# OnurBasci/TransformerBasedNavierStokeSolver

Measured on AMD Instinct MI355X. Metric: ns64_train_samples_per_s, higher is better.
Workload: dtype f32

## Files before the change

transformerbasednavierstokesolver_amd/csrc/pa2d_gemm.hip:

```cpp
#include "pa2d_gemm_common.h"
#include <string.h>


static Pa2dEnv read_env() {
    auto is = [](const char* n, const char* pre) { const char* e = getenv(n); return e && strncmp(e, pre, strlen(pre)) == 0; };
    auto num = [](const char* n, int dflt) { const char* e = getenv(n); return (e && e[0]) ? atoi(e) : dflt; };
    Pa2dEnv v;
    v.conv_halo = is("PA2D_CONV_HALO", "o") ? 0 : (is("PA2D_CONV_HALO", "f") ? 2 : 1);
    v.mc_big_off = is("PA2D_MC_BIG", "o") ? 1 : 0;
    v.kc_bk16 = num("PA2D_KC_BK", 0) == 16 ? 1 : 0;
    v.mc_bk = num("PA2D_MC_BK", 16) == 32 ? 32 : 16;
    v.mc_splits = num("PA2D_MC_SPLITS", 0);
    v.mcb_splits = num("PA2D_MCB_SPLITS", 0);
    v.lin_dw_split = is("PA2D_LIN_DW_SPLIT", "of") ? 0 : 1;
    v.lin_panel = is("PA2D_LIN_PANEL", "of") ? 0 : 1;
    v.lin_rowpanel = is("PA2D_LIN_ROWPANEL", "of") ? 0 : 1;
    v.lin_small_split = is("PA2D_LIN_SMALL_SPLIT", "of") ? 0 : 1;
    v.conv_mfma16 = num("PA2D_CONV_MFMA", 16) == 32 ? 0 : 1;
    v.conv_ahead = num("PA2D_CONV_AHEAD", 1) == 0 ? 0 : 1;
    v.mc_mfma16 = num("PA2D_MC_MFMA", 16) == 32 ? 0 : 1;
    v.mc_dma = num("PA2D_MC_DMA", 1) == 0 ? 0 : 1;
    v.mc_chain = num("PA2D_MC_CHAIN", 1) == 0 ? 0 : 1;
    v.split_big = num("PA2D_SPLIT_BIG", 1);
    v.slice_map = is("PA2D_SLICE_MAP", "l") ? 0 : 1;
    v.default_engine = is("PA2D_GEMM", "f") ? 0 : (is("PA2D_GEMM", "b") ? 2 : 1);
    v.tail_panel = num("PA2D_TAIL_PANEL", 0);
    return v;
}
static Pa2dEnv g_env = read_env();
const Pa2dEnv& pa2d_env() { return g_env; }


static int kc_bk(bool im2col, int Cin) {
    if (im2col && pa2d_env().kc_bk16) return 16;
    return (!im2col || (Cin % 32) == 0) ? 32 : 16;
}
static KCTile kc_tile(int M, int N, bool im2col, int Cin) {
    const int tiles_m = ceil_div(M, 128);
    const long long t128 = (long long)tiles_m * ceil_div(N, 128);
    const long long t12864 = (long long)tiles_m * ceil_div(N, 64);
    const int bk = kc_bk(im2col, Cin);
    if (N > 64 && t128 >= 384) return {128, 128, bk};
    if (t12864 >= 384 || M <= 64) return {128, 64, bk};
    return {64, 64, bk};
}
static bool use_split(int engine, int N, bool im2col, int Cin) {
    const int m = engine;
    if (m == 1) return im2col && N > 64 && (Cin % 32) == 0;
    if (m == 2) return N > 64 && (!im2col || (Cin % 32) == 0);
    return false;
}
static bool kc_split_small_applies(const KCParams& p, bool im2col) {
    if (!pa2d_env().lin_small_split || im2col || p.io_bf16 || p.engine != 1) return false;
    if ((p.K % 32) != 0 || p.K < 64 || p.N < 64 || p.M < 256) return false;
    return (long long)ceil_div(p.M, 128) * ceil_div(p.N, 128) < 384;
}
static int persistent_mode(const KCParams& p) {
    const bool gelu = p.act == ACT_GELU, has_res = p.res != nullptr;
    if (p.epi == 0) return 0;
    if (gelu && !has_res && (p.epi == (EPI_ACT | EPI_STORE_PRE) || p.epi == EPI_ACT)) return 1;
    if (gelu && !has_res && p.epi == EPI_MUL_DACT && !p.bias) return 2;
    return -1;
}
static bool panel_applies(const KCParams& p, bool im2col) {
    if (!pa2d_env().lin_panel || im2col) return false;
    if (p.io_bf16 || (p.engine != 1 && p.engine != 2)) return false;
    if ((p.K % 32) != 0 || p.N < 64) return false;
    if (persistent_mode(p) < 0) return false;
    if (p.epi == EPI_ACT && p.aux) return false;
    return (long long)(p.M / 256) * ceil_div(p.N, 128) >= 256;
}
static size_t rowpanel_image_bytes(int N, int K, int engine) {
    if (engine != 1 || (K != 128 && K != 256) || N < 128 || N > 1024 || (N % 128) != 0) return 0;
    return (size_t)N * K * 6;
}
static bool rowpanel_applies(const KCParams& p) {
    if (!pa2d_env().lin_rowpanel || p.io_bf16) return false;
    if (rowpanel_image_bytes(p.N, p.K, p.engine) == 0) return false;
    if (persistent_mode(p) < 0 || (p.epi == EPI_ACT && p.aux)) return false;
    if ((p.lda & 3) || (p.ldc & 3) || (p.res && (p.ldres & 3)) || (p.aux && (p.ldaux & 3))) return false;
    return p.M / 128 >= 256;
}
static bool conv_halo_applies(const KCParams& p) {
    const int pol = pa2d_env().conv_halo;
    if (p.taps == 27) return false;
    if (pol == 0 || !p.apre || (p.Cin % 32) != 0 || p.H <= 0 || p.W <= 0 || (p.M % (p.H * p.W)) != 0) return false;
    const long long tiles = (long long)(p.M / (p.H * p.W)) * ceil_div(p.H, KC_HALO_TH) * ceil_div(p.W, KC_HALO_TW) * ceil_div(p.N, 128);
    return pol == 2 || tiles >= 512;
}

KCChoice plan_kc(const KCParams& p, bool im2col) {
    KCChoice c = {};
    c.mode = c.tail_family = c.tail_bm = c.tail_bn = -1;
    c.out_bf16 = p.io_bf16;
    c.reads_b = true;
    c.wimg_bytes = im2col ? 0 : rowpanel_image_bytes(p.N, p.K, p.engine);
    const int nt = p.engine == 2 ? 1 : 3;
    if (!im2col && p.wimg && rowpanel_applies(p)) {
        c.family = KC_ROWPANEL; c.bm = 128; c.bn = 64; c.bk = 64; c.nt = 3;
    } else if (panel_applies(p, im2col)) {
        c.family = KC_PANEL; c.bm = 256; c.bn = 128; c.bk = 32; c.nt = nt;
    } else if (p.io_bf16 || use_split(p.engine, p.N, im2col, p.Cin)) {
        c.family = KC_SPLIT; c.bm = 128; c.bn = 128; c.bk = 32; c.nt = nt;
        c.a_planes = im2col ? p.apre != 0 : p.io_bf16 != 0;
        if (im2col) c.pack = KC_PACK_PLANES;
        if (im2col ? !p.apre : p.engine != 2) c.rc = PA2D_ERR_ARG;
        else if (p.io_bf16 && (p.taps == 27 || p.engine != 2 || (!im2col && (p.K % 32) != 0))) c.rc = PA2D_ERR_UNSUPPORTED;
        else if (im2col && conv_halo_applies(p)) {
            c.family = KC_HALO; c.bm = 256;
            c.mfma16 = nt == 3 && pa2d_env().conv_mfma16 && (p.N % 4) == 0 && (p.ldc % 4) == 0;
            c.ahead = c.mfma16 && pa2d_env().conv_ahead;
        } else if (im2col && !p.io_bf16 && nt == 3) {
            const int tiles_n = ceil_div(p.N, 128);
            if (pa2d_env().split_big && (p.M % 256) == 0 && (long long)(p.M / 256) * tiles_n >= 512) c.bm = 256;
            else if ((long long)ceil_div(p.M, 128) * tiles_n < 256) c.bm = 64;
        }
    } else if (kc_split_small_applies(p, im2col)) {
        c.family = KC_SPLIT_SMALL; c.bm = 64; c.bn = 64; c.bk = 32; c.nt = 3;
    } else {
        const KCTile t = kc_tile(p.M, p.N, im2col, p.Cin);
        c.family = KC_EXACT; c.bm = t.bm; c.bn = t.bn; c.bk = t.bk;
        if (im2col) c.pack = t.bk == 32 ? KC_PACK_F32_32 : KC_PACK_F32_16;
    }
    if (c.family == KC_PANEL || c.family == KC_ROWPANEL) {
        c.mode = persistent_mode(p);
        c.head_rows = p.M - p.M % c.bm;
        if (c.head_rows < p.M) {
            KCParams pt = p;
            pt.wimg = nullptr;
            pt.M = p.M - c.head_rows;
            const KCChoice t = plan_kc(pt, false);
            c.tail_family = t.family; c.tail_bm = t.bm; c.tail_bn = t.bn;
        }
        c.reads_b = c.family == KC_PANEL || c.head_rows < p.M;
    }
    return c;
}

static bool kc_extents(KCParams& p, bool im2col, const KCChoice& c) {
    const unsigned long long lim = 0xFFFFFFF0ull;
    const unsigned long long es = p.io_bf16 ? 2ull : 4ull;
    unsigned long long ab = ((unsigned long long)(p.M - 1) * p.lda + (im2col ? p.Cin : p.K)) * 4ull;
    unsigned long long bb = ((unsigned long long)(p.N - 1) * p.ldb + p.K) * 4ull;
    const unsigned long long cb = ((unsigned long long)(p.M - 1) * p.ldc + p.N) * es;
    const unsigned long long rb = p.res ? ((unsigned long long)(p.M - 1) * p.ldres + p.N) * es : 0ull;
    const unsigned long long xb = p.aux ? ((unsigned long long)(p.M - 1) * p.ldaux + p.N) * es : 0ull;
    if (ab >= lim || bb >= lim || cb >= lim || rb >= lim || xb >= lim) return false;
    if (c.a_planes) ab = im2col ? (unsigned long long)p.M * (p.Cin / 32) * c.nt * 64 : ab / 2;
    if (c.pack == KC_PACK_PLANES) bb = (unsigned long long)p.N * (p.K / 32) * c.nt * 64;
    if (ab >= lim) return false;
    p.a_bytes = (unsigned)ab; p.b_bytes = (unsigned)bb;
    p.c_bytes = (unsigned)cb; p.res_bytes = (unsigned)rb; p.aux_bytes = (unsigned)xb;
    return true;
}

static int launch_head_tail(const KCParams& p_in, const KCParams& p, const KCChoice& c, hipStream_t st) {
    int rc;
    if (c.family == KC_ROWPANEL && p.wsrc) {
        rc = launch_pack_weight_image(p.wsrc, p.wsn, p.wsk, p.wimg, p.N, p.K, st);
        if (rc) return rc;
    }
    KCParams ph = p;
    ph.M = c.head_rows;
    rc = c.family == KC_ROWPANEL ? launch_kc_rowpanel(ph, c, st) : launch_kc_panel(ph, c, st);
    if (rc || c.head_rows == p.M) return rc;
    KCParams pt = p_in;
    pt.wimg = nullptr;
    pt.M = p.M - c.head_rows;
    pt.A = p.A + (size_t)c.head_rows * p.lda;
    pt.C = p.C + (size_t)c.head_rows * p.ldc;
    if (p.res) pt.res = p.res + (size_t)c.head_rows * p.ldres;
    if (p.aux) pt.aux = p.aux + (size_t)c.head_rows * p.ldaux;
    return launch_kc(pt, false, st);
}

// ... 258 lines not shown
```

transformerbasednavierstokesolver_amd/csrc/pa2d_gemm_rowpanel.hip:

```cpp
#include "pa2d_gemm_common.h"
#include <type_traits>
#ifndef RP_SGB
#define RP_SGB 1
#endif

namespace {

constexpr int RP_STAGE = 24 * 1024;
constexpr int RP_SLOTS = 3;
constexpr int RP_BIAS = 4096;

typedef unsigned int u32x4_ __attribute__((ext_vector_type(4)));

__device__ __forceinline__ float4 ld4s(__amdgpu_buffer_rsrc_t r, unsigned voff, unsigned soff) {
    const u32x4_ v = __builtin_amdgcn_raw_buffer_load_b128(r, voff, soff, 0);
    return make_float4(__uint_as_float(v.x), __uint_as_float(v.y), __uint_as_float(v.z), __uint_as_float(v.w));
}
__device__ __forceinline__ void st4s(__amdgpu_buffer_rsrc_t r, unsigned voff, unsigned soff, const float (&v)[4]) {
    const u32x4_ u = {__float_as_uint(v[0]), __float_as_uint(v[1]), __float_as_uint(v[2]), __float_as_uint(v[3])};
    __builtin_amdgcn_raw_buffer_store_b128(u, r, voff, soff, 0);
}
__device__ __forceinline__ bf16x8 cat8(bf16x4 a, bf16x4 b) { return __builtin_shufflevector(a, b, 0, 1, 2, 3, 4, 5, 6, 7); }

__global__ void pack_weight_image_kernel(const float* __restrict__ src, long long sn, long long sk, unsigned char* __restrict__ img,
                                         int N, int K) {
    const int idx = blockIdx.x * blockDim.x + threadIdx.x;
    const int KC = K / 64;
    if (idx >= (N / 64) * KC * 8 * 64) return;
    const int lane = idx & 63, j = (idx >> 6) & 1, sub = (idx >> 7) & 3, stage = idx >> 9;
    const int np = stage / KC, kc = stage % KC;
    const int n = 64 * np + 16 * (2 * (sub & 1) + j) + (lane & 15), k0 = 64 * kc + 32 * (sub >> 1) + 8 * (lane >> 4);
    float v[8];
#pragma unroll
    for (int e = 0; e < 8; ++e) v[e] = src[(long long)n * sn + (long long)(k0 + e) * sk];
    bf16x4 h0, m0, l0, h1, m1, l1;
    split3(make_float4(v[0], v[1], v[2], v[3]), h0, m0, l0);
    split3(make_float4(v[4], v[5], v[6], v[7]), h1, m1, l1);
    unsigned char* dst = img + (size_t)stage * RP_STAGE + (size_t)((sub * 2 + j) * 3) * 1024 + lane * 16;
    *reinterpret_cast<bf16x8*>(dst) = cat8(h0, h1);
    *reinterpret_cast<bf16x8*>(dst + 1024) = cat8(m0, m1);
    *reinterpret_cast<bf16x8*>(dst + 2048) = cat8(l0, l1);
}

template <int KS, int MODE, bool HAS_RES>
__global__ __launch_bounds__(256, 1) void gemm_rowpanel_kernel(const KCParams p, const unsigned char* __restrict__ img,
                                                               const unsigned img_bytes) {
    constexpr int KC = KS / 4;
    extern __shared__ __attribute__((aligned(16))) unsigned char smem[];
    const int tid = threadIdx.x, lane = tid & 63;
    const int wave = __builtin_amdgcn_readfirstlane(tid >> 6);
    const int li = lane & 15, kq = lane >> 4;
    const int NP = p.N / 64, SPR = NP * KC;
    float* const bias_s = reinterpret_cast<float*>(smem);
    unsigned char* const ring = smem + RP_BIAS;
    for (int c = tid; c < p.N; c += 256)
        bias_s[c] = (MODE != 2 && p.bias) ? (c < p.bias_split ? p.bias[c] : p.bias2[c - p.bias_split]) : 0.f;
    const int rounds = p.M / 128;
    const int n_my = ((int)blockIdx.x < rounds) ? (rounds - (int)blockIdx.x + (int)gridDim.x - 1) / (int)gridDim.x : 0;
    if (n_my == 0) return;
    const int T = n_my * SPR;

    const __amdgpu_buffer_rsrc_t ra = make_rsrc(p.A, p.a_bytes);
    const __amdgpu_buffer_rsrc_t ri = make_rsrc_v(img, img_bytes);
    const __amdgpu_buffer_rsrc_t rc = make_rsrc(p.C, p.c_bytes);
    const __amdgpu_buffer_rsrc_t rres = make_rsrc(p.res ? p.res : p.C, p.res ? p.res_bytes : 0u);
    const __amdgpu_buffer_rsrc_t raux = make_rsrc(p.aux ? p.aux : p.C, p.aux ? p.aux_bytes : 0u);
    const unsigned lda_b = (unsigned)p.lda * 4u, ldc_b = (unsigned)p.ldc * 4u, ldres_b = (unsigned)p.ldres * 4u,
                   ldaux_b = (unsigned)p.ldaux * 4u;

    const unsigned piece = (unsigned)(wave * 6) * 1024u + (unsigned)lane * 16u;
    u32x4_ breg[6];
    int ld_stage = 0;
    auto stage_load = [&]() {
#pragma unroll
        for (int i = 0; i < 6; ++i)
            breg[i] = __builtin_amdgcn_raw_buffer_load_b128(ri, piece + i * 1024u, (unsigned)ld_stage * RP_STAGE, 0);
        if (++ld_stage == SPR) ld_stage = 0;
    };
    auto stage_write = [&](int slot) {
#pragma unroll
        for (int i = 0; i < 6; ++i) *reinterpret_cast<u32x4_*>(ring + slot * RP_STAGE + piece + i * 1024) = breg[i];
    };

    const unsigned a_voff = (unsigned)li * lda_b + (unsigned)kq * 32u;
    float4 raw[KS][2];
    bf16x8 ap[KS][3];
    auto a_load = [&](int u, unsigned voff, unsigned row0) {
        const unsigned so = (row0 + 16u * (u & 1)) * lda_b;
        raw[u][0] = ld4s(ra, voff == OOB_OFF ? OOB_OFF : voff + (u >> 1) * 128u, so);
        raw[u][1] = ld4s(ra, voff == OOB_OFF ? OOB_OFF : voff + (u >> 1) * 128u + 16u, so);
    };
    auto a_split = [&](int ks) {
        bf16x4 h0, m0, l0, h1, m1, l1;
        split3(raw[ks][0], h0, m0, l0);
        split3(raw[ks][1], h1, m1, l1);
        ap[ks][0] = cat8(h0, h1); ap[ks][1] = cat8(m0, m1); ap[ks][2] = cat8(l0, l1);
    };

    int round = blockIdx.x;
    unsigned row0 = (unsigned)(round * 128 + wave * 32);
#pragma unroll
    for (int ks = 0; ks < KS; ++ks) a_load(ks, a_voff, row0);
    stage_load();
    stage_write(0);
    stage_load();
#pragma unroll
    for (int ks = 0; ks < KS; ++ks) a_split(ks);
    __syncthreads();

    const unsigned vc = li * ldc_b + kq * 16u, vr = li * ldres_b + kq * 16u, vx = li * ldaux_b + kq * 16u;

    bf16x8 bfb[2][2][3];
    int cur = 0;
    auto frag_read = [&](int buf, int slot, int ks4) {
        const unsigned char* bs = ring + slot * RP_STAGE + lane * 16;
#pragma unroll
        for (int j = 0; j < 2; ++j)
#pragma unroll
            for (int u = 0; u < 3; ++u) bfb[buf][j][u] = *reinterpret_cast<const bf16x8*>(bs + ((ks4 * 2 + j) * 3 + u) * 1024);
    };
    frag_read(0, 0, 0);

    f32x4 acc[2][4];
    float4 ov[2][4];
    auto ep_group = [&](const int q8, const int np) {
        const int rb = q8 >> 2, nt = q8 & 3;
        const unsigned cb = (unsigned)(np * 64 + nt * 16) * 4u;
        const unsigned rw = row0 + 16u * rb;
        float v[4];
#pragma unroll
        for (int e = 0; e < 4; ++e) v[e] = acc[rb][nt][e];
        if (MODE == 1) {
            if (p.aux_deriv) {
                float d[4];
#pragma unroll
                for (int e = 0; e < 4; ++e) d[e] = dgelu_f(v[e]);
                st4s(raux, vx, rw * ldaux_b + cb, d);
            } else {
                st4s(raux, vx, rw * ldaux_b + cb, v);
            }
#pragma unroll
            for (int e = 0; e < 4; ++e) v[e] = gelu_f(v[e]);
        } else if (MODE == 2) {
            if (p.aux_deriv) {
                v[0] *= ov[rb][nt].x; v[1] *= ov[rb][nt].y; v[2] *= ov[rb][nt].z; v[3] *= ov[rb][nt].w;
            } else {
                v[0] *= dgelu_f(ov[rb][nt].x); v[1] *= dgelu_f(ov[rb][nt].y); v[2] *= dgelu_f(ov[rb][nt].z); v[3] *= dgelu_f(ov[rb][nt].w);
            }
        } else if (HAS_RES) {
            v[0] += ov[rb][nt].x; v[1] += ov[rb][nt].y; v[2] += ov[rb][nt].z; v[3] += ov[rb][nt].w;
        }
#ifdef RP_NO_STORE
        if (p.M == 12345)
#endif
        st4s(rc, vc, rw * ldc_b + cb, v);
    };
    auto ov_load = [&](const int q8, const int np) {
        const int rb = q8 >> 2, nt = q8 & 3;
        const unsigned cb = (unsigned)(np * 64 + nt * 16) * 4u;
        if (MODE == 2) ov[rb][nt] = ld4s(raux, vx, (row0 + 16u * rb) * ldaux_b + cb);
        else if (HAS_RES) ov[rb][nt] = ld4s(rres, vr, (row0 + 16u * rb) * ldres_b + cb);
    };

    unsigned row0n = 0, a_voff_n = OOB_OFF;
    auto pair = [&](auto first_tag, auto last_tag, const int np) {
        constexpr bool FIRST = decltype(first_tag)::value, LAST = decltype(last_tag)::value;
#pragma unroll
        for (int nt = 0; nt < 4; ++nt) {
            const float4 bv = *reinterpret_cast<const float4*>(bias_s + np * 64 + nt * 16 + 4 * kq);
#pragma unroll
            for (int rb = 0; rb < 2; ++rb) {
                acc[rb][nt] = f32x4{bv.x, bv.y, bv.z, bv.w};
                ov_load(rb * 4 + nt, np);
            }
        }
#pragma unroll
        for (int kc = 0; kc < KC; ++kc) {
            const int nxt = cur == 2 ? 0 : cur + 1;
#ifndef RP_NO_BSTAGE
            stage_write(nxt);
            stage_load();
#endif
#ifndef RP_NO_ANEXT
            if (FIRST) {
#pragma unroll
                for (int q = 0; q < 4; ++q) a_load(kc * 4 + q, a_voff_n, row0n);
            }
#endif
#pragma unroll
            for (int ks4 = 0; ks4 < 4; ++ks4) {
                if (ks4 < 3) frag_read((ks4 + 1) & 1, cur, ks4 + 1);
                else frag_read(0, nxt, 0);
#if RP_SGB == 2
                __builtin_amdgcn_sched_barrier(0);
#endif
                const int ks = kc * 4 + ks4;
#ifndef RP_NO_ANEXT
                if (LAST && kc >= 1) a_split(ks - 4);
                if (FIRST && kc == 0) a_split(KS - 4 + ks4);
#endif
#define RP_MFMA(u_, v_)                                                                                      \
    _Pragma("unroll") for (int j = 0; j < 2; ++j) _Pragma("unroll") for (int rb = 0; rb < 2; ++rb)            \
        acc[rb][2 * (ks4 & 1) + j] = __builtin_amdgcn_mfma_f32_16x16x32_bf16(                                 \
            bfb[ks4 & 1][j][v_], ap[kc * 4 + (ks4 >> 1) * 2 + rb][u_], acc[rb][2 * (ks4 & 1) + j], 0, 0, 0);
#ifndef RP_NO_MFMA
                RP_MFMA(1, 1) RP_MFMA(2, 0) RP_MFMA(0, 2) RP_MFMA(1, 0) RP_MFMA(0, 1) RP_MFMA(0, 0)
#endif
#undef RP_MFMA
#if RP_SGB == 1
#pragma unroll
                for (int i = 0; i < 6; ++i) {
                    __builtin_amdgcn_sched_group_barrier(0x008, 4, 0);
                    __builtin_amdgcn_sched_group_barrier(0x100, 1, 0);
                }
#endif
#ifndef RP_NO_BARRIER
                if (ks4 == 1) __syncthreads();
#endif
            }
            cur = nxt;
        }
#pragma unroll
        for (int q8 = 0; q8 < 8; ++q8) ep_group(q8, np);
    };
    using T_ = std::true_type; using F_ = std::false_type;

    for (int t = 0; t < n_my; ++t) {
        const bool more = t + 1 < n_my;
        row0n = more ? (unsigned)((round + (int)gridDim.x) * 128 + wave * 32) : 0u;
        a_voff_n = more ? a_voff : OOB_OFF;
        pair(T_{}, F_{}, 0);
        for (int np = 1; np < NP - 1; ++np) pair(F_{}, F_{}, np);
        pair(F_{}, T_{}, NP - 1);
        round += gridDim.x;
        row0 = row0n;
    }
}

template <int KS, int MODE, bool HAS_RES>
int launch_rowpanel_t(const KCParams& p, hipStream_t st) {
    const int smem = RP_BIAS + RP_SLOTS * RP_STAGE;
    const int rounds = p.M / 128;
    const unsigned img_bytes = (unsigned)((size_t)p.N * p.K * 6);
    return launch_lds(&gemm_rowpanel_kernel<KS, MODE, HAS_RES>, dim3(rounds < 256 ? rounds : 256), dim3(256), smem, st, p,
                      (const unsigned char*)p.wimg, img_bytes);
}

template <int KS>
int launch_rowpanel_k(const KCParams& p, int mode, hipStream_t st) {
    switch (mode) {
        case 0: return p.res ? launch_rowpanel_t<KS, 0, true>(p, st) : launch_rowpanel_t<KS, 0, false>(p, st);
        case 1: return launch_rowpanel_t<KS, 1, false>(p, st);
        case 2: return launch_rowpanel_t<KS, 2, false>(p, st);
        default: return PA2D_ERR_ARG;
    }
}

}

int launch_pack_weight_image(const float* w, long long sn, long long sk, void* img, int N, int K, hipStream_t st) {
    const int count = (N / 64) * (K / 64) * 8 * 64;
    hipLaunchKernelGGL(pack_weight_image_kernel, dim3(ceil_div(count, 256)), dim3(256), 0, st, w, sn, sk, (unsigned char*)img, N, K);
    PA2D_CHECK_LAUNCH();
    return PA2D_OK;
}

int launch_kc_rowpanel(const KCParams& p, const KCChoice& c, hipStream_t st) {
    return p.K == 256 ? launch_rowpanel_k<16>(p, c.mode, st) : launch_rowpanel_k<8>(p, c.mode, st);
}
```

transformerbasednavierstokesolver_amd/csrc/pa2d_internal.h:

```cpp
#pragma once
#include <hip/hip_runtime.h>
#include <stdint.h>

typedef float f32x16 __attribute__((ext_vector_type(16)));
typedef float f32x4 __attribute__((ext_vector_type(4)));

#define PA2D_OK 0
#define PA2D_ERR_ARG 1001
#define PA2D_ERR_UNSUPPORTED 1002
#define PA2D_ERR_WORKSPACE 1003

#define PA2D_CHECK_LAUNCH()                         \
    do {                                            \
        hipError_t e__ = hipGetLastError();         \
        if (e__ != hipSuccess) return (int)e__;     \
    } while (0)

enum { ACT_NONE = 0, ACT_GELU = 1, ACT_TANH = 2, ACT_SIGMOID = 3, ACT_RELU = 4, ACT_SOFTPLUS = 5,
       ACT_ELU = 6, ACT_SILU = 7 };

__device__ __forceinline__ float normal_cdf(float x, float& e_out) {
#pragma clang fp contract(off)
    const float z = fabsf(x) * 0.70710678118654752440f;
    const float t = __builtin_amdgcn_rcpf(fmaf(0.3275911f, z, 1.0f));
    float poly = fmaf(1.061405429f, t, -1.453152027f);
    poly = fmaf(poly, t, 1.421413741f);
    poly = fmaf(poly, t, -0.284496736f);
    poly = fmaf(poly, t, 0.254829592f);
    const float e = __builtin_amdgcn_exp2f(-z * z * 1.44269504088896340736f);
    e_out = e;
    const float hq = 0.5f * poly * t * e;
    return x < 0.f ? hq : 1.0f - hq;
}
__device__ __forceinline__ float gelu_exact(float x) {
#pragma clang fp contract(off)
    float e;
    return x * normal_cdf(x, e);
}
__device__ __forceinline__ float dgelu_exact(float x) {
#pragma clang fp contract(off)
    float e;
    const float cdf = normal_cdf(x, e);
    return fmaf(x * 0.39894228040143267794f, e, cdf);
}

__device__ __forceinline__ float act_fwd(int id, float x) {
    switch (id) {
        case ACT_GELU: return gelu_exact(x);
        case ACT_TANH: return tanhf(x);
        case ACT_SIGMOID: return 1.0f / (1.0f + expf(-x));
        case ACT_RELU: return x > 0.f ? x : 0.f;
        case ACT_SOFTPLUS: return x > 20.f ? x : log1pf(expf(x));
        case ACT_ELU: return x > 0.f ? x : expm1f(x);
        case ACT_SILU: return x / (1.0f + expf(-x));
        default: return x;
    }
}

__device__ __forceinline__ float act_bwd(int id, float x) {
    switch (id) {
        case ACT_GELU: return dgelu_exact(x);
        case ACT_TANH: { const float t = tanhf(x); return 1.0f - t * t; }
        case ACT_SIGMOID: { const float s = 1.0f / (1.0f + expf(-x)); return s * (1.0f - s); }
        case ACT_RELU: return x > 0.f ? 1.f : 0.f;
        case ACT_SOFTPLUS: return x > 20.f ? 1.f : 1.0f / (1.0f + expf(-x));
        case ACT_ELU: return x > 0.f ? 1.f : expf(x);
        case ACT_SILU: { const float s = 1.0f / (1.0f + expf(-x)); return s * (1.0f + x * (1.0f - s)); }
        default: return 1.f;
    }
}

__device__ __forceinline__ float wave_sum(float v) {
#pragma unroll
    for (int o = 32; o > 0; o >>= 1) v += __shfl_xor(v, o, 64);
    return v;
}
__device__ __forceinline__ float wave_max(float v) {
#pragma unroll
    for (int o = 32; o > 0; o >>= 1) v = fmaxf(v, __shfl_xor(v, o, 64));
    return v;
}

typedef unsigned int u32x4 __attribute__((ext_vector_type(4)));
#define OOB_OFF 0xFFFFFFFFu

__device__ __forceinline__ __amdgpu_buffer_rsrc_t make_rsrc(const float* base, unsigned bytes) {
    return __builtin_amdgcn_make_buffer_rsrc(const_cast<float*>(base), 0, bytes, 0x00020000);
}
__device__ __forceinline__ float4 buf_load4(__amdgpu_buffer_rsrc_t r, unsigned voff) {
    const u32x4 v = __builtin_amdgcn_raw_buffer_load_b128(r, voff, 0, 0);
    return make_float4(__uint_as_float(v.x), __uint_as_float(v.y), __uint_as_float(v.z), __uint_as_float(v.w));
}


__device__ __forceinline__ float buf_load1(__amdgpu_buffer_rsrc_t r, unsigned voff) {
    return __uint_as_float(__builtin_amdgcn_raw_buffer_load_b32(r, voff, 0, 0));
}
__device__ __forceinline__ void buf_store1(__amdgpu_buffer_rsrc_t r, unsigned voff, float v) {
    __builtin_amdgcn_raw_buffer_store_b32(__float_as_uint(v), r, voff, 0, 0);
}

__device__ __forceinline__ float2 buf_load2(__amdgpu_buffer_rsrc_t r, unsigned voff) {
    typedef unsigned int u32x2_ __attribute__((ext_vector_type(2)));
    const u32x2_ v = __builtin_amdgcn_raw_buffer_load_b64(r, voff, 0, 0);
    return make_float2(__uint_as_float(v.x), __uint_as_float(v.y));
}
__device__ __forceinline__ void buf_store4(__amdgpu_buffer_rsrc_t r, unsigned voff, float4 v) {
    u32x4 u = {__float_as_uint(v.x), __float_as_uint(v.y), __float_as_uint(v.z), __float_as_uint(v.w)};
    __builtin_amdgcn_raw_buffer_store_b128(u, r, voff, 0, 0);
}

#define PA2D_ACT_SAVE_DERIVATIVE_BIT 0x100

struct Pa2dEnv {
    int conv_halo;
    int mc_big_off;
    int kc_bk16;
    int mc_bk;
    int mc_splits;
    int mcb_splits;
    int lin_dw_split;
    int lin_panel;
    int conv_mfma16;
    int conv_ahead;
    int mc_mfma16;
    int mc_dma;
    int mc_chain;
    int lin_small_split;
    int lin_rowpanel;
    int split_big;
    int slice_map;
    int default_engine;
    int tail_panel;
};
const Pa2dEnv& pa2d_env();

static inline int pa2d_zero(void* p, size_t bytes, hipStream_t st) {
    if (!p || !bytes) return PA2D_OK;
    return (int)hipMemsetAsync(p, 0, bytes, st);
}
static inline int ceil_div(int a, int b) { return (a + b - 1) / b; }
static inline long long ceil_div_ll(long long a, long long b) { return (a + b - 1) / b; }

struct ReduceSegs { int nseg; long long begin[5]; float* dst[4]; };
int pa2d_launch_reduce_segs(const float* slab, int nslab, long long count, const ReduceSegs& segs, int accumulate,
                            hipStream_t st);

typedef __bf16 bf16_t;
template <typename T> struct Act;
template <> struct Act<float> {
    static constexpr unsigned ES = 4;
    static __device__ __forceinline__ float4 ld4(const float* p) { return *reinterpret_cast<const float4*>(p); }
    static __device__ __forceinline__ void st4(float* p, float4 v) { *reinterpret_cast<float4*>(p) = v; }
    static __device__ __forceinline__ float ld1(const float* p) { return *p; }
    static __device__ __forceinline__ float4 bld4(__amdgpu_buffer_rsrc_t r, unsigned off) { return buf_load4(r, off); }
    static __device__ __forceinline__ float2 bld2(__amdgpu_buffer_rsrc_t r, unsigned off) { return buf_load2(r, off); }
    static __device__ __forceinline__ float bld1(__amdgpu_buffer_rsrc_t r, unsigned off) { return buf_load1(r, off); }
    static __device__ __forceinline__ float bld1s(__amdgpu_buffer_rsrc_t r, unsigned off, unsigned soff) {
        return __uint_as_float(__builtin_amdgcn_raw_buffer_load_b32(r, off, soff, 0));
    }
    static __device__ __forceinline__ void bst4(__amdgpu_buffer_rsrc_t r, unsigned off, float4 v) { buf_store4(r, off, v); }
    static __device__ __forceinline__ void bst1(__amdgpu_buffer_rsrc_t r, unsigned off, float v) { buf_store1(r, off, v); }
};
__device__ __forceinline__ float bf16_bits_to_f32(unsigned short b) { return __uint_as_float((unsigned)b << 16); }
__device__ __forceinline__ unsigned short f32_to_bf16_bits(float x) {
    const bf16_t h = (bf16_t)x;
    return __builtin_bit_cast(unsigned short, h);
}
__device__ __forceinline__ unsigned pack_bf16x2(float lo, float hi) {
    return (unsigned)f32_to_bf16_bits(lo) | ((unsigned)f32_to_bf16_bits(hi) << 16);
}
template <> struct Act<bf16_t> {
    static constexpr unsigned ES = 2;
    static __device__ __forceinline__ float4 unpack4(uint2 q) {
        return make_float4(__uint_as_float(q.x << 16), __uint_as_float(q.x & 0xFFFF0000u), __uint_as_float(q.y << 16),
                           __uint_as_float(q.y & 0xFFFF0000u));
    }
    static __device__ __forceinline__ float4 ld4(const bf16_t* p) { return unpack4(*reinterpret_cast<const uint2*>(p)); }
    static __device__ __forceinline__ void st4(bf16_t* p, float4 v) {
        *reinterpret_cast<uint2*>(p) = make_uint2(pack_bf16x2(v.x, v.y), pack_bf16x2(v.z, v.w));
    }
    static __device__ __forceinline__ float ld1(const bf16_t* p) { return (float)*p; }
    static __device__ __forceinline__ float4 bld4(__amdgpu_buffer_rsrc_t r, unsigned off) {
        typedef unsigned int u32x2_ __attribute__((ext_vector_type(2)));
        const u32x2_ q = __builtin_amdgcn_raw_buffer_load_b64(r, off, 0, 0);
        return unpack4(make_uint2(q.x, q.y));
    }
    static __device__ __forceinline__ float2 bld2(__amdgpu_buffer_rsrc_t r, unsigned off) {
        const unsigned q = __builtin_amdgcn_raw_buffer_load_b32(r, off, 0, 0);
        return make_float2(__uint_as_float(q << 16), __uint_as_float(q & 0xFFFF0000u));
    }
    static __device__ __forceinline__ float bld1(__amdgpu_buffer_rsrc_t r, unsigned off) {
        return bf16_bits_to_f32(__builtin_amdgcn_raw_buffer_load_b16(r, off, 0, 0));
    }
    static __device__ __forceinline__ float bld1s(__amdgpu_buffer_rsrc_t r, unsigned off, unsigned soff) {
        return bf16_bits_to_f32(__builtin_amdgcn_raw_buffer_load_b16(r, off, soff, 0));
    }
    static __device__ __forceinline__ void bst4(__amdgpu_buffer_rsrc_t r, unsigned off, float4 v) {
        typedef unsigned int u32x2_ __attribute__((ext_vector_type(2)));
        const u32x2_ q = {pack_bf16x2(v.x, v.y), pack_bf16x2(v.z, v.w)};
        __builtin_amdgcn_raw_buffer_store_b64(q, r, off, 0, 0);
    }
    static __device__ __forceinline__ void bst1(__amdgpu_buffer_rsrc_t r, unsigned off, float v) {
        __builtin_amdgcn_raw_buffer_store_b16(f32_to_bf16_bits(v), r, off, 0, 0);
    }
};
__device__ __forceinline__ __amdgpu_buffer_rsrc_t make_rsrc_v(const void* base, unsigned bytes) {
    return __builtin_amdgcn_make_buffer_rsrc(const_cast<void*>(base), 0, bytes, 0x00020000);
}

__device__ __forceinline__ bool slice_decode(int xcd_map, int B, int heads, int nchunk, int& b, int& hh, int& chunk, int& bid) {
    const int total = B * heads * nchunk;
    int L;
    if (xcd_map) {
        const int per = (total + 7) >> 3;
        if ((int)(blockIdx.x >> 3) >= per) return false;
        L = (int)(blockIdx.x & 7) * per + (int)(blockIdx.x >> 3);
        if (L >= total) return false;
        hh = L % heads;
        chunk = (L / heads) % nchunk;
        b = L / (heads * nchunk);
    } else {
        L = (int)blockIdx.x;
        if (L >= total) return false;
        chunk = L % nchunk;
        hh = (L / nchunk) % heads;
        b = L / (nchunk * heads);
    }
    bid = (b * heads + hh) * nchunk + chunk;
    return true;
}
static inline int slice_grid(int total) { return ((total + 7) / 8) * 8; }
```

Measured before the change: 72.30.

## Stage rowpanel GEMM weight tiles via buffer-load-to-LDS DMA with chained fragment reads

Adds a path in the row-panel GEMM kernel that loads the packed weight image straight into the LDS ring with buffer_load ... lds instructions, instead of staging it through VGPRs and writing it to LDS. A chained variant splits the B-fragment reads per tile and interleaves them between MFMA runs using scheduling barriers. Freeing the staging registers and the LDS write instructions is meant to cut VGPR pressure and LDS-store traffic and to let loads overlap compute. The cost is hand-written inline asm with manual m0 handling and hand-tuned vmcnt counts, which could break correctness if the outstanding-load accounting is wrong. Both paths are on by default.

Result: no change. 72.96, median of 6 (+0.9%).

```diff
diff --git a/transformerbasednavierstokesolver_amd/csrc/pa2d_gemm.hip b/transformerbasednavierstokesolver_amd/csrc/pa2d_gemm.hip
--- a/transformerbasednavierstokesolver_amd/csrc/pa2d_gemm.hip
+++ b/transformerbasednavierstokesolver_amd/csrc/pa2d_gemm.hip
@@ -21,6 +21,8 @@
     v.mc_mfma16 = num("PA2D_MC_MFMA", 16) == 32 ? 0 : 1;
     v.mc_dma = num("PA2D_MC_DMA", 1) == 0 ? 0 : 1;
     v.mc_chain = num("PA2D_MC_CHAIN", 1) == 0 ? 0 : 1;
+    v.rp_dma = num("PA2D_RP_DMA", 1) == 0 ? 0 : 1;
+    v.rp_chain = (v.rp_dma && num("PA2D_RP_CHAIN", 1) != 0) ? 1 : 0;
     v.split_big = num("PA2D_SPLIT_BIG", 1);
     v.slice_map = is("PA2D_SLICE_MAP", "l") ? 0 : 1;
     v.default_engine = is("PA2D_GEMM", "f") ? 0 : (is("PA2D_GEMM", "b") ? 2 : 1);
diff --git a/transformerbasednavierstokesolver_amd/csrc/pa2d_gemm_rowpanel.hip b/transformerbasednavierstokesolver_amd/csrc/pa2d_gemm_rowpanel.hip
--- a/transformerbasednavierstokesolver_amd/csrc/pa2d_gemm_rowpanel.hip
+++ b/transformerbasednavierstokesolver_amd/csrc/pa2d_gemm_rowpanel.hip
@@ -42,9 +42,10 @@
     *reinterpret_cast<bf16x8*>(dst + 2048) = cat8(l0, l1);
 }
 
-template <int KS, int MODE, bool HAS_RES>
+template <int KS, int MODE, bool HAS_RES, bool DMA = false, bool CHAIN = false>
 __global__ __launch_bounds__(256, 1) void gemm_rowpanel_kernel(const KCParams p, const unsigned char* __restrict__ img,
                                                                const unsigned img_bytes) {
+    static_assert(!CHAIN || DMA, "the chained issue order needs the registers that DMA staging frees");
     constexpr int KC = KS / 4;
     extern __shared__ __attribute__((aligned(16))) unsigned char smem[];
     const int tid = threadIdx.x, lane = tid & 63;
@@ -69,7 +70,7 @@
                    ldaux_b = (unsigned)p.ldaux * 4u;
 
     const unsigned piece = (unsigned)(wave * 6) * 1024u + (unsigned)lane * 16u;
-    u32x4_ breg[6];
+    u32x4_ breg[DMA ? 1 : 6];
     int ld_stage = 0;
     auto stage_load = [&]() {
 #pragma unroll
@@ -81,6 +82,31 @@
 #pragma unroll
         for (int i = 0; i < 6; ++i) *reinterpret_cast<u32x4_*>(ring + slot * RP_STAGE + piece + i * 1024) = breg[i];
     };
+#define RP_DMA_ASM                                                                                        \
+    "s_nop 4\n\ts_mov_b32 %0, m0\n\ts_mov_b32 m0, %1\n\ts_nop 0\n\t"                                      \
+    "buffer_load_dwordx4 %3, %2, 0 offen lds\n\ts_add_u32 m0, m0, 0x400\n\ts_nop 0\n\t"                   \
+    "buffer_load_dwordx4 %4, %2, 0 offen lds\n\ts_add_u32 m0, m0, 0x400\n\ts_nop 0\n\t"                   \
+    "buffer_load_dwordx4 %5, %2, 0 offen lds\n\ts_add_u32 m0, m0, 0x400\n\ts_nop 0\n\t"                   \
+    "buffer_load_dwordx4 %6, %2, 0 offen lds\n\ts_add_u32 m0, m0, 0x400\n\ts_nop 0\n\t"                   \
+    "buffer_load_dwordx4 %7, %2, 0 offen lds\n\ts_add_u32 m0, m0, 0x400\n\ts_nop 0\n\t"                   \
+    "buffer_load_dwordx4 %8, %2, 0 offen lds\n\ts_mov_b32 m0, %0"
+    typedef __attribute__((address_space(3))) unsigned char lds_char;
+    const unsigned lds_ring = (unsigned)(uintptr_t)(lds_char*)smem + (unsigned)RP_BIAS + (unsigned)(wave * 6) * 1024u;
+    const u32x4_ dma_ri = {(unsigned)(uintptr_t)img, (unsigned)((uintptr_t)img >> 32) & 0xFFFFu, img_bytes, 0x00020000u};
+    auto stage_dma = [&](int slot) {
+        const unsigned so = piece + (unsigned)ld_stage * RP_STAGE;
+        unsigned keep;
+        asm volatile(RP_DMA_ASM
+                     : "=&s"(keep)
+                     : "s"(lds_ring + (unsigned)slot * (unsigned)RP_STAGE), "s"(dma_ri), "v"(so), "v"(so + 1024u), "v"(so + 2048u),
+                       "v"(so + 3072u), "v"(so + 4096u), "v"(so + 5120u)
+                     : "memory", "scc");
+        if (++ld_stage == SPR) ld_stage = 0;
+    };
+#undef RP_DMA_ASM
+#ifndef RP_DMA_WAIT
+#define RP_DMA_WAIT 1
+#endif
 
     const unsigned a_voff = (unsigned)li * lda_b + (unsigned)kq * 32u;
     float4 raw[KS][2];
@@ -101,11 +127,17 @@
     unsigned row0 = (unsigned)(round * 128 + wave * 32);
 #pragma unroll
     for (int ks = 0; ks < KS; ++ks) a_load(ks, a_voff, row0);
-    stage_load();
-    stage_write(0);
-    stage_load();
+    if constexpr (DMA) {
+        stage_dma(0);
+        stage_dma(1);
+    } else {
+        stage_load();
+        stage_write(0);
+        stage_load();
+    }
 #pragma unroll
     for (int ks = 0; ks < KS; ++ks) a_split(ks);
+    if constexpr (DMA) asm volatile("s_waitcnt vmcnt(0)" ::: "memory");
     __syncthreads();
 
     const unsigned vc = li * ldc_b + kq * 16u, vr = li * ldres_b + kq * 16u, vx = li * ldaux_b + kq * 16u;
@@ -119,7 +151,13 @@
 #pragma unroll
             for (int u = 0; u < 3; ++u) bfb[buf][j][u] = *reinterpret_cast<const bf16x8*>(bs + ((ks4 * 2 + j) * 3 + u) * 1024);
     };
+    auto frag_read_tile = [&](int buf, int slot, int ks4, int j) {
+        const unsigned char* bs = ring + slot * RP_STAGE + lane * 16;
+#pragma unroll
+        for (int u = 0; u < 3; ++u) bfb[buf][j][u] = *reinterpret_cast<const bf16x8*>(bs + ((ks4 * 2 + j) * 3 + u) * 1024);
+    };
     frag_read(0, 0, 0);
+    if constexpr (CHAIN) frag_read_tile(1, 0, 1, 0);
 
     f32x4 acc[2][4];
     float4 ov[2][4];
@@ -178,8 +216,10 @@
         for (int kc = 0; kc < KC; ++kc) {
             const int nxt = cur == 2 ? 0 : cur + 1;
 #ifndef RP_NO_BSTAGE
-            stage_write(nxt);
-            stage_load();
+            if constexpr (!DMA) {
+                stage_write(nxt);
+                stage_load();
+            }
 #endif
 #ifndef RP_NO_ANEXT
             if (FIRST) {
@@ -189,8 +229,14 @@
 #endif
 #pragma unroll
             for (int ks4 = 0; ks4 < 4; ++ks4) {
+                if constexpr (CHAIN) {
+                    if (ks4 < 3) frag_read_tile((ks4 + 1) & 1, cur, ks4 + 1, 1);
+                    else frag_read_tile(0, nxt, 0, 1);
+                    __builtin_amdgcn_sched_barrier(0);
+                } else {
                 if (ks4 < 3) frag_read((ks4 + 1) & 1, cur, ks4 + 1);
                 else frag_read(0, nxt, 0);
+                }
 #if RP_SGB == 2
                 __builtin_amdgcn_sched_barrier(0);
 #endif
@@ -199,23 +245,54 @@
                 if (LAST && kc >= 1) a_split(ks - 4);
                 if (FIRST && kc == 0) a_split(KS - 4 + ks4);
 #endif
+#define RP_MFMA1(u_, v_, j_, rb_)                                                                            \
+        acc[rb_][2 * (ks4 & 1) + j_] = __builtin_amdgcn_mfma_f32_16x16x32_bf16(                               \
+            bfb[ks4 & 1][j_][v_], ap[kc * 4 + (ks4 >> 1) * 2 + rb_][u_], acc[rb_][2 * (ks4 & 1) + j_], 0, 0, 0);
 #define RP_MFMA(u_, v_)                                                                                      \
-    _Pragma("unroll") for (int j = 0; j < 2; ++j) _Pragma("unroll") for (int rb = 0; rb < 2; ++rb)            \
-        acc[rb][2 * (ks4 & 1) + j] = __builtin_amdgcn_mfma_f32_16x16x32_bf16(                                 \
-            bfb[ks4 & 1][j][v_], ap[kc * 4 + (ks4 >> 1) * 2 + rb][u_], acc[rb][2 * (ks4 & 1) + j], 0, 0, 0);
+    _Pragma("unroll") for (int j = 0; j < 2; ++j) _Pragma("unroll") for (int rb = 0; rb < 2; ++rb) RP_MFMA1(u_, v_, j, rb)
+#define RP_RUN(j_, rb_)                                                                                      \
+    RP_MFMA1(1, 1, j_, rb_) RP_MFMA1(2, 0, j_, rb_) RP_MFMA1(0, 2, j_, rb_) RP_MFMA1(1, 0, j_, rb_) RP_MFMA1(0, 1, j_, rb_) \
+    RP_MFMA1(0, 0, j_, rb_) __builtin_amdgcn_sched_barrier(0);
 #ifndef RP_NO_MFMA
+                if constexpr (CHAIN) {
+                    RP_RUN(0, 0) RP_RUN(0, 1)
+                    if (ks4 < 2) frag_read_tile(ks4 & 1, cur, ks4 + 2, 0);
+                    else frag_read_tile(ks4 & 1, nxt, ks4 - 2, 0);
+                    __builtin_amdgcn_sched_barrier(0);
+                    RP_RUN(1, 0) RP_RUN(1, 1)
+                } else {
                 RP_MFMA(1, 1) RP_MFMA(2, 0) RP_MFMA(0, 2) RP_MFMA(1, 0) RP_MFMA(0, 1) RP_MFMA(0, 0)
-#endif
+                }
+#endif
+#undef RP_RUN
 #undef RP_MFMA
+#undef RP_MFMA1
 #if RP_SGB == 1
+                if constexpr (!CHAIN) {
 #pragma unroll
                 for (int i = 0; i < 6; ++i) {
                     __builtin_amdgcn_sched_group_barrier(0x008, 4, 0);
                     __builtin_amdgcn_sched_group_barrier(0x100, 1, 0);
                 }
+                }
 #endif
 #ifndef RP_NO_BARRIER
-                if (ks4 == 1) __syncthreads();
+                if (ks4 == 1) {
+                    if constexpr (DMA) {
+#if RP_DMA_WAIT == 1 && !defined(RP_NO_STORE) && !defined(RP_NO_ANEXT)
+                        constexpr int A_NEXT = FIRST ? 8 : 0;
+                        constexpr int N0 = (MODE == 1 ? 16 : 8) + ((MODE == 2 || HAS_RES) ? 8 : 0) + A_NEXT;
+                        if (kc == 0) asm volatile("s_waitcnt vmcnt(%0)" ::"n"(N0) : "memory");
+                        else asm volatile("s_waitcnt vmcnt(%0)" ::"n"(A_NEXT) : "memory");
+#else
+                        asm volatile("s_waitcnt vmcnt(0)" ::: "memory");
+#endif
+                    }
+                    __syncthreads();
+#ifndef RP_NO_BSTAGE
+                    if constexpr (DMA) stage_dma(cur == 0 ? 2 : cur - 1);
+#endif
+                }
 #endif
             }
             cur = nxt;
@@ -235,6 +312,7 @@
         round += gridDim.x;
         row0 = row0n;
     }
+    if constexpr (DMA) asm volatile("s_waitcnt vmcnt(0)" ::: "memory");
 }
 
 template <int KS, int MODE, bool HAS_RES>
@@ -242,8 +320,12 @@
     const int smem = RP_BIAS + RP_SLOTS * RP_STAGE;
     const int rounds = p.M / 128;
     const unsigned img_bytes = (unsigned)((size_t)p.N * p.K * 6);
-    return launch_lds(&gemm_rowpanel_kernel<KS, MODE, HAS_RES>, dim3(rounds < 256 ? rounds : 256), dim3(256), smem, st, p,
-                      (const unsigned char*)p.wimg, img_bytes);
+    const dim3 grid(rounds < 256 ? rounds : 256);
+    const unsigned char* img = (const unsigned char*)p.wimg;
+    const int dma = pa2d_env().rp_dma ? (pa2d_env().rp_chain ? 2 : 1) : 0;
+    if (dma == 2) return launch_lds(&gemm_rowpanel_kernel<KS, MODE, HAS_RES, true, true>, grid, dim3(256), smem, st, p, img, img_bytes);
+    if (dma == 1) return launch_lds(&gemm_rowpanel_kernel<KS, MODE, HAS_RES, true>, grid, dim3(256), smem, st, p, img, img_bytes);
+    return launch_lds(&gemm_rowpanel_kernel<KS, MODE, HAS_RES>, grid, dim3(256), smem, st, p, img, img_bytes);
 }
 
 template <int KS>
diff --git a/transformerbasednavierstokesolver_amd/csrc/pa2d_internal.h b/transformerbasednavierstokesolver_amd/csrc/pa2d_internal.h
--- a/transformerbasednavierstokesolver_amd/csrc/pa2d_internal.h
+++ b/transformerbasednavierstokesolver_amd/csrc/pa2d_internal.h
@@ -126,6 +126,8 @@
     int mc_mfma16;
     int mc_dma;
     int mc_chain;
+    int rp_dma;
+    int rp_chain;
     int lin_small_split;
     int lin_rowpanel;
     int split_big;
```

## Pipeline rowpanel B-fragment reads through a 4-slot ring and stage residuals in LDS

Applied to the files above, without the earlier changes.

Replaces the two-buffer B-fragment read in the rowpanel GEMM with a 4-unit register ring that prefetches three units ahead, including across stage slots. MFMA chains are grouped per row block with sched_group_barrier hints that interleave LDS reads and MFMAs. For the K=256 residual and backward-GELU epilogues, the residual/aux values are loaded early and parked in 32KB of extra LDS instead of registers, which lowers register pressure. Environment flags select the new arms, and the extra LDS and scheduler pinning may change latency hiding.

Result: no change. 71.29 before, 71.06 after (-0.3%).

```diff
diff --git a/transformerbasednavierstokesolver_amd/csrc/pa2d_gemm.hip b/transformerbasednavierstokesolver_amd/csrc/pa2d_gemm.hip
--- a/transformerbasednavierstokesolver_amd/csrc/pa2d_gemm.hip
+++ b/transformerbasednavierstokesolver_amd/csrc/pa2d_gemm.hip
@@ -21,6 +21,8 @@
     v.mc_mfma16 = num("PA2D_MC_MFMA", 16) == 32 ? 0 : 1;
     v.mc_dma = num("PA2D_MC_DMA", 1) == 0 ? 0 : 1;
     v.mc_chain = num("PA2D_MC_CHAIN", 1) == 0 ? 0 : 1;
+    v.rp_ring = num("PA2D_RP_RING", 1) == 0 ? 0 : 1;
+    v.rp_chain = num("PA2D_RP_CHAIN", 1) == 0 ? 0 : 1;
     v.split_big = num("PA2D_SPLIT_BIG", 1);
     v.slice_map = is("PA2D_SLICE_MAP", "l") ? 0 : 1;
     v.default_engine = is("PA2D_GEMM", "f") ? 0 : (is("PA2D_GEMM", "b") ? 2 : 1);
diff --git a/transformerbasednavierstokesolver_amd/csrc/pa2d_gemm_rowpanel.hip b/transformerbasednavierstokesolver_amd/csrc/pa2d_gemm_rowpanel.hip
--- a/transformerbasednavierstokesolver_amd/csrc/pa2d_gemm_rowpanel.hip
+++ b/transformerbasednavierstokesolver_amd/csrc/pa2d_gemm_rowpanel.hip
@@ -3,12 +3,20 @@
 #ifndef RP_SGB
 #define RP_SGB 1
 #endif
+#ifndef RP_CHAIN_PIN
+#define RP_CHAIN_PIN 1
+#endif
 
 namespace {
 
 constexpr int RP_STAGE = 24 * 1024;
 constexpr int RP_SLOTS = 3;
 constexpr int RP_BIAS = 4096;
+constexpr int RP_OV = 32 * 1024;
+
+constexpr bool rp_ov_lds(int KS, int MODE, bool HAS_RES, int ARM) {
+    return KS == 16 && ((ARM >= 1 && HAS_RES) || (ARM == 2 && MODE == 2));
+}
 
 typedef unsigned int u32x4_ __attribute__((ext_vector_type(4)));
 
@@ -42,7 +50,7 @@
     *reinterpret_cast<bf16x8*>(dst + 2048) = cat8(l0, l1);
 }
 
-template <int KS, int MODE, bool HAS_RES>
+template <int KS, int MODE, bool HAS_RES, int ARM>
 __global__ __launch_bounds__(256, 1) void gemm_rowpanel_kernel(const KCParams p, const unsigned char* __restrict__ img,
                                                                const unsigned img_bytes) {
     constexpr int KC = KS / 4;
@@ -53,6 +61,8 @@
     const int NP = p.N / 64, SPR = NP * KC;
     float* const bias_s = reinterpret_cast<float*>(smem);
     unsigned char* const ring = smem + RP_BIAS;
+    constexpr bool OV_LDS = rp_ov_lds(KS, MODE, HAS_RES, ARM);
+    unsigned char* const ov_s = smem + RP_BIAS + RP_SLOTS * RP_STAGE + wave * (RP_OV / 4) + lane * 16;
     for (int c = tid; c < p.N; c += 256)
         bias_s[c] = (MODE != 2 && p.bias) ? (c < p.bias_split ? p.bias[c] : p.bias2[c - p.bias_split]) : 0.f;
     const int rounds = p.M / 128;
@@ -110,16 +120,25 @@
 
     const unsigned vc = li * ldc_b + kq * 16u, vr = li * ldres_b + kq * 16u, vx = li * ldaux_b + kq * 16u;
 
-    bf16x8 bfb[2][2][3];
+    bf16x8 bfb[4][3];
     int cur = 0;
     auto frag_read = [&](int buf, int slot, int ks4) {
         const unsigned char* bs = ring + slot * RP_STAGE + lane * 16;
 #pragma unroll
         for (int j = 0; j < 2; ++j)
 #pragma unroll
-            for (int u = 0; u < 3; ++u) bfb[buf][j][u] = *reinterpret_cast<const bf16x8*>(bs + ((ks4 * 2 + j) * 3 + u) * 1024);
-    };
-    frag_read(0, 0, 0);
+            for (int u = 0; u < 3; ++u) bfb[2 * buf + j][u] = *reinterpret_cast<const bf16x8*>(bs + ((ks4 * 2 + j) * 3 + u) * 1024);
+    };
+    auto unit_read = [&](int slot, int u8) {
+        const unsigned char* bs = ring + slot * RP_STAGE + lane * 16 + u8 * 3 * 1024;
+#pragma unroll
+        for (int u = 0; u < 3; ++u) bfb[u8 & 3][u] = *reinterpret_cast<const bf16x8*>(bs + u * 1024);
+    };
+    if constexpr (ARM == 0) {
+        frag_read(0, 0, 0);
+    } else {
+        unit_read(0, 0); unit_read(0, 1); unit_read(0, 2);
+    }
 
     f32x4 acc[2][4];
     float4 ov[2][4];
@@ -142,12 +161,14 @@
 #pragma unroll
             for (int e = 0; e < 4; ++e) v[e] = gelu_f(v[e]);
         } else if (MODE == 2) {
+            if constexpr (OV_LDS) ov[rb][nt] = *reinterpret_cast<const float4*>(ov_s + q8 * 1024);
             if (p.aux_deriv) {
                 v[0] *= ov[rb][nt].x; v[1] *= ov[rb][nt].y; v[2] *= ov[rb][nt].z; v[3] *= ov[rb][nt].w;
             } else {
                 v[0] *= dgelu_f(ov[rb][nt].x); v[1] *= dgelu_f(ov[rb][nt].y); v[2] *= dgelu_f(ov[rb][nt].z); v[3] *= dgelu_f(ov[rb][nt].w);
             }
         } else if (HAS_RES) {
+            if constexpr (OV_LDS) ov[rb][nt] = *reinterpret_cast<const float4*>(ov_s + q8 * 1024);
             v[0] += ov[rb][nt].x; v[1] += ov[rb][nt].y; v[2] += ov[rb][nt].z; v[3] += ov[rb][nt].w;
         }
 #ifdef RP_NO_STORE
@@ -171,7 +192,7 @@
 #pragma unroll
             for (int rb = 0; rb < 2; ++rb) {
                 acc[rb][nt] = f32x4{bv.x, bv.y, bv.z, bv.w};
-                ov_load(rb * 4 + nt, np);
+                if constexpr (!OV_LDS) ov_load(rb * 4 + nt, np);
             }
         }
 #pragma unroll
@@ -179,6 +200,18 @@
             const int nxt = cur == 2 ? 0 : cur + 1;
 #ifndef RP_NO_BSTAGE
             stage_write(nxt);
+#endif
+            if constexpr (OV_LDS) {
+                if (kc == 1 || kc == 2) {
+#pragma unroll
+                    for (int nt = 0; nt < 4; ++nt) *reinterpret_cast<float4*>(ov_s + ((kc - 1) * 4 + nt) * 1024) = ov[kc - 1][nt];
+                }
+                if (kc < 2) {
+#pragma unroll
+                    for (int nt = 0; nt < 4; ++nt) ov_load(kc * 4 + nt, np);
+                }
+            }
+#ifndef RP_NO_BSTAGE
             stage_load();
 #endif
 #ifndef RP_NO_ANEXT
@@ -187,6 +220,7 @@
                 for (int q = 0; q < 4; ++q) a_load(kc * 4 + q, a_voff_n, row0n);
             }
 #endif
+            if constexpr (ARM == 0) {
 #pragma unroll
             for (int ks4 = 0; ks4 < 4; ++ks4) {
                 if (ks4 < 3) frag_read((ks4 + 1) & 1, cur, ks4 + 1);
@@ -202,7 +236,7 @@
 #define RP_MFMA(u_, v_)                                                                                      \
     _Pragma("unroll") for (int j = 0; j < 2; ++j) _Pragma("unroll") for (int rb = 0; rb < 2; ++rb)            \
         acc[rb][2 * (ks4 & 1) + j] = __builtin_amdgcn_mfma_f32_16x16x32_bf16(                                 \
-            bfb[ks4 & 1][j][v_], ap[kc * 4 + (ks4 >> 1) * 2 + rb][u_], acc[rb][2 * (ks4 & 1) + j], 0, 0, 0);
+            bfb[2 * (ks4 & 1) + j][v_], ap[kc * 4 + (ks4 >> 1) * 2 + rb][u_], acc[rb][2 * (ks4 & 1) + j], 0, 0, 0);
 #ifndef RP_NO_MFMA
                 RP_MFMA(1, 1) RP_MFMA(2, 0) RP_MFMA(0, 2) RP_MFMA(1, 0) RP_MFMA(0, 1) RP_MFMA(0, 0)
 #endif
@@ -217,6 +251,49 @@
 #ifndef RP_NO_BARRIER
                 if (ks4 == 1) __syncthreads();
 #endif
+            }
+            } else {
+#pragma unroll
+            for (int u8 = 0; u8 < 8; ++u8) {
+                const int ks4 = u8 >> 1, j = u8 & 1;
+                if (u8 + 3 < 8) unit_read(cur, u8 + 3);
+                else unit_read(nxt, u8 - 5);
+#if RP_CHAIN_PIN == 2
+                if (ARM == 2) __builtin_amdgcn_sched_barrier(0);
+#endif
+#ifndef RP_NO_ANEXT
+                if (j == 0) {
+                    const int ks = kc * 4 + ks4;
+                    if (LAST && kc >= 1) a_split(ks - 4);
+                    if (FIRST && kc == 0) a_split(KS - 4 + ks4);
+                }
+#endif
+#define RP_UMFMA(rb_, u_, v_)                                                                                \
+    acc[rb_][2 * (ks4 & 1) + j] = __builtin_amdgcn_mfma_f32_16x16x32_bf16(                                   \
+        bfb[u8 & 3][v_], ap[kc * 4 + (ks4 >> 1) * 2 + rb_][u_], acc[rb_][2 * (ks4 & 1) + j], 0, 0, 0);
+#define RP_UCHAIN(rb_) RP_UMFMA(rb_, 1, 1) RP_UMFMA(rb_, 2, 0) RP_UMFMA(rb_, 0, 2) RP_UMFMA(rb_, 1, 0) RP_UMFMA(rb_, 0, 1) RP_UMFMA(rb_, 0, 0)
+                if constexpr (ARM == 1) {
+                    RP_UCHAIN(0) RP_UCHAIN(1)
+#pragma unroll
+                    for (int i = 0; i < 3; ++i) {
+                        __builtin_amdgcn_sched_group_barrier(0x008, 4, 0);
+                        __builtin_amdgcn_sched_group_barrier(0x100, 1, 0);
+                    }
+                } else {
+#if RP_CHAIN_PIN == 2
+                    RP_UCHAIN(0) __builtin_amdgcn_sched_barrier(0);
+                    RP_UCHAIN(1) __builtin_amdgcn_sched_barrier(0);
+#else
+                    RP_UCHAIN(0) RP_UCHAIN(1)
+                    __builtin_amdgcn_sched_group_barrier(0x100, 3, 0);
+                    __builtin_amdgcn_sched_group_barrier(0x008, 6, 0);
+                    __builtin_amdgcn_sched_group_barrier(0x008, 6, 0);
+#endif
+                }
+#undef RP_UCHAIN
+#undef RP_UMFMA
+                if (u8 == 3) __syncthreads();
+            }
             }
             cur = nxt;
         }
@@ -237,23 +314,27 @@
     }
 }
 
-template <int KS, int MODE, bool HAS_RES>
+template <int KS, int MODE, bool HAS_RES, int ARM>
 int launch_rowpanel_t(const KCParams& p, hipStream_t st) {
-    const int smem = RP_BIAS + RP_SLOTS * RP_STAGE;
+    const int smem = RP_BIAS + RP_SLOTS * RP_STAGE + (rp_ov_lds(KS, MODE, HAS_RES, ARM) ? RP_OV : 0);
     const int rounds = p.M / 128;
     const unsigned img_bytes = (unsigned)((size_t)p.N * p.K * 6);
-    return launch_lds(&gemm_rowpanel_kernel<KS, MODE, HAS_RES>, dim3(rounds < 256 ? rounds : 256), dim3(256), smem, st, p,
+    return launch_lds(&gemm_rowpanel_kernel<KS, MODE, HAS_RES, ARM>, dim3(rounds < 256 ? rounds : 256), dim3(256), smem, st, p,
                       (const unsigned char*)p.wimg, img_bytes);
 }
 
-template <int KS>
+template <int KS, int ARM>
 int launch_rowpanel_k(const KCParams& p, int mode, hipStream_t st) {
     switch (mode) {
-        case 0: return p.res ? launch_rowpanel_t<KS, 0, true>(p, st) : launch_rowpanel_t<KS, 0, false>(p, st);
-        case 1: return launch_rowpanel_t<KS, 1, false>(p, st);
-        case 2: return launch_rowpanel_t<KS, 2, false>(p, st);
+        case 0: return p.res ? launch_rowpanel_t<KS, 0, true, ARM>(p, st) : launch_rowpanel_t<KS, 0, false, ARM>(p, st);
+        case 1: return launch_rowpanel_t<KS, 1, false, ARM>(p, st);
+        case 2: return launch_rowpanel_t<KS, 2, false, ARM>(p, st);
         default: return PA2D_ERR_ARG;
     }
+}
+template <int ARM>
+int launch_rowpanel_a(const KCParams& p, int mode, hipStream_t st) {
+    return p.K == 256 ? launch_rowpanel_k<16, ARM>(p, mode, st) : launch_rowpanel_k<8, ARM>(p, mode, st);
 }
 
 }
@@ -266,5 +347,7 @@
 }
 
 int launch_kc_rowpanel(const KCParams& p, const KCChoice& c, hipStream_t st) {
-    return p.K == 256 ? launch_rowpanel_k<16>(p, c.mode, st) : launch_rowpanel_k<8>(p, c.mode, st);
-}
+    if (!pa2d_env().rp_ring) return launch_rowpanel_a<0>(p, c.mode, st);
+    if (pa2d_env().rp_chain) return launch_rowpanel_a<2>(p, c.mode, st);
+    return launch_rowpanel_a<1>(p, c.mode, st);
+}
diff --git a/transformerbasednavierstokesolver_amd/csrc/pa2d_internal.h b/transformerbasednavierstokesolver_amd/csrc/pa2d_internal.h
--- a/transformerbasednavierstokesolver_amd/csrc/pa2d_internal.h
+++ b/transformerbasednavierstokesolver_amd/csrc/pa2d_internal.h
@@ -128,6 +128,8 @@
     int mc_chain;
     int lin_small_split;
     int lin_rowpanel;
+    int rp_ring;
+    int rp_chain;
     int split_big;
     int slice_map;
     int default_engine;
```
